# LJacksonPan/RaTrack

Measured on AMD Instinct MI355X. Metric: radar frame-pairs/sec (backbone forward, eval) at B=64,N=256 per GPU, higher is better.
Workload: dtype f32 (2xfp16 split MFMA: three fp16 products per fp32 product, fp32 accumulate, power-of-two scales per matrix and position); 1 GPU; Track4D.backbone forward, B=64 frame-pairs x N=256 points per GPU, S=512 centroids, eval-mode BN, random-init weights, hipGraph=True, batches in flight=4; global_batch=64, parallelism=replicas x1 (no collective on the forward path)

## Files before the change

include/rtk_fused.h:

```cpp
#ifndef RTK_FUSED_H
#define RTK_FUSED_H

#include "rtk_pointnet2.h"

#ifdef __cplusplus
extern "C" {
#endif

#define RTK_MAX_SRC 4
#define RTK_MAX_LAYERS 4

typedef struct {
    const float *ptr;
    int pitch;
    int channels;
    int per_sample;
} rtk_src_t;

#define RTK_LAYER_SPLIT 0x100
typedef struct {
    const float *w_packed;
    const float *bias;
    int cin16, cout16;
    int act;
// ... 82 lines not shown
    float *out;
    int cout, s0, count, out_pitch;
    const float *wt2;
    int s2;
} rtk_gterm_job_t;
RTK_EXPORT int rtk_global_terms(int samples, int cin, const float *g, int njobs, const rtk_gterm_job_t *jobs, float *bcast, int bcast_pitch,
                                int n, rtk_stream_t stream);

#define RTK_COPY_MAX_JOBS 8
typedef struct {
    const void *src;
    void *dst;
    long bytes;
} rtk_copy_job_t;
RTK_EXPORT int rtk_copy_multi(int njobs, const rtk_copy_job_t *jobs, rtk_stream_t stream);

RTK_EXPORT int rtk_to_channel_major(int samples, int n, int channels, const float *src, int src_pitch, int per_sample,
                                    float *dst, int dst_channels, int dst_channel_offset, rtk_stream_t stream);

RTK_EXPORT int rtk_ball_query_pair(int b, int n, int npoint, float radius1, int nsample1, float radius2, int nsample2,
                                   const float *new_xyz, const float *xyz, int *idx1, int *idx2, const int *nuniq,
                                   rtk_stream_t stream);

RTK_EXPORT int rtk_three_nn_masked(int b, int n, int m, const float *unknown, const float *known, float *dist2, int *idx,
                                   const int *unknown_nuniq, const int *known_nuniq, rtk_stream_t stream);

RTK_EXPORT int rtk_geometry_front(int b, int clouds, int n, int npoint, const float *frame1, const float *frame2, int channel_major,
                                  const float *feature1, const float *feature2, float *xyz, float *raw, int *fps_idx, float *new_xyz,
                                  int *nuniq, int *tie, int *first_tie, float *snap, const int *n_valid, int64_t *knn12, int64_t *knn11,
                                  const float *q1_w, float *q1_out, int q1_cout, rtk_stream_t stream);
RTK_EXPORT int rtk_geometry_tables(int samples, int n, int npoint, const float *xyz0, const float *new_xyz, const int *nuniq,
                                   const float *radii, const int *nsamples, int *const *ball, int *const *nn_idx, float *const *nn_dist2,
                                   rtk_stream_t stream);

typedef struct {
    const float *src; float *dst;
    int channels, src_pitch, per_sample, dst_channels, dst_channel_offset;
} rtk_layout_job_t;
RTK_EXPORT int rtk_to_channel_major_multi(int samples, int n, int njobs, const rtk_layout_job_t *jobs, rtk_stream_t stream);

RTK_EXPORT int rtk_log_sinkhorn(int m, int n, const float *scores, float alpha, int iters, float *out, rtk_stream_t stream);

RTK_EXPORT int rtk_dbscan(int n, const float *feat, int pitch, const int *channels, const float *score, float threshold, double eps,
                          int min_samples, int *labels, rtk_stream_t stream);

#define RTK_DESC 141

typedef struct {
    const float *ptr;
    long long sb, sc, sp;
} rtk_bcn_view_t;

typedef struct {
    int B, N;
    rtk_bcn_view_t pc1, flow, feature1, prop, cls;
    const int *n_valid;
    const unsigned char *active;
} rtk_track_frame_t;

#define RTK_DBSCAN_POINT_BYTES 48
RTK_EXPORT int rtk_dbscan_batched(const rtk_track_frame_t *frame, float threshold, double eps, int min_samples, int K, int *labels,
                                  int *obj, int *num_objects, int *flags, void *work, long long work_bytes, rtk_stream_t stream);

RTK_EXPORT int rtk_object_descriptors(const rtk_track_frame_t *frame, int K, const int *obj, const int *num_objects,
                                      const int *prev_count, const float *desc_prev, float *desc, rtk_stream_t stream);

// ... 17 lines not shown
```

ratrack_amd/csrc/ops_pointnet2.hip:

```cpp
#include <math.h>
#include <stdarg.h>
#include <string.h>

#include "rtk_common.h"
#include "rtk_fused.h"

static thread_local char g_err[512] = "";

void rtk_set_error(const char *fmt, ...) {
    va_list ap;
    va_start(ap, fmt);
    vsnprintf(g_err, sizeof(g_err), fmt, ap);
    va_end(ap);
}

extern "C" const char *rtk_last_error(void) { return g_err; }
extern "C" int rtk_version(void) { return (0 << 16) | 3; }

template <int CTRL, int ROW_MASK>
__device__ __forceinline__ unsigned dpp_max_u32(unsigned v) {
    const unsigned o = (unsigned)__builtin_amdgcn_update_dpp(0, (int)v, CTRL, ROW_MASK, 0xf, true);
    return v > o ? v : o;
}

// ... 404 lines not shown
                const float py = USE_LDS ? sy[k] : xyz[k * 3 + 1];
                const float pz = USE_LDS ? sz[k] : xyz[k * 3 + 2];
                hit = rtk_sqdist(qx, qy, qz, px, py, pz) < radius2;
            }
            const unsigned long long mask = __ballot(hit);
            if (mask) {
                if (first < 0) first = base + __builtin_ctzll(mask);
                const int rank = cnt + __builtin_popcountll(mask & ((1ull << lane) - 1ull));
                if (hit && rank < nsample) out[rank] = k;
                cnt += __builtin_popcountll(mask);
            }
        }
        if (first >= 0 && cnt < nsample) {
            for (int l = cnt + lane; l < nsample; l += 64) out[l] = first;
        }
    }
}

extern "C" int rtk_ball_query(int b, int n, int npoint, float radius, int nsample, const float *new_xyz,
                              const float *xyz, int *idx, rtk_stream_t stream) {
    RTK_REQUIRE(b > 0 && n > 0 && npoint > 0 && nsample > 0 && new_xyz && xyz && idx, "ball_query: bad arguments");
    RTK_REQUIRE(b <= 65535, "ball_query: b exceeds grid limits");
    const float r2 = radius * radius;
    dim3 grid(rtk_divup(npoint, BQ_WAVES * BQ_CENTROIDS_PER_WAVE), b);
    const size_t lds = (size_t)n * 3 * sizeof(float);
    if (lds <= 64 * 1024)
        ball_query_kernel<true><<<grid, 64 * BQ_WAVES, lds, (hipStream_t)stream>>>(n, npoint, r2, nsample, new_xyz, xyz, idx);
    else
        ball_query_kernel<false><<<grid, 64 * BQ_WAVES, 0, (hipStream_t)stream>>>(n, npoint, r2, nsample, new_xyz, xyz, idx);
    RTK_CHECK_LAUNCH("ball_query");
    return RTK_OK;
}

__device__ __forceinline__ void ball_query_pair_body(int bs, int chunk0, int chunk_stride, int n, int m, float r2a, int nsa, float r2b, int nsb,
                                                     const float *__restrict__ new_xyz, const float *__restrict__ xyz,
                                                     int *__restrict__ idxa, int *__restrict__ idxb, const int *__restrict__ nuniq,
                                                     float *smem, const int *__restrict__ src_nuniq = nullptr) {
    const int tid = threadIdx.x, wave = tid >> 6, lane = tid & 63;
    constexpr int CPC = BQ_WAVES * BQ_CENTROIDS_PER_WAVE;
    xyz += (size_t)bs * n * 3;
    float *sx = smem, *sy = smem + n, *sz = smem + 2 * n;
    const int climit = nuniq ? min(m, nuniq[bs]) : m;
    if (chunk0 * CPC >= climit) return;
    const int n_full = n;
    if (src_nuniq) n = max(1, min(n, src_nuniq[bs]));
    if (chunk0 == 0) {
        const int z1 = min(m, (climit + 31) & ~31);
        int *za = idxa + ((size_t)bs * m + climit) * nsa, *zb = idxb + ((size_t)bs * m + climit) * nsb;
        for (int l = tid; l < (z1 - climit) * nsa; l += 64 * BQ_WAVES) za[l] = 0;
        for (int l = tid; l < (z1 - climit) * nsb; l += 64 * BQ_WAVES) zb[l] = 0;
    }
    for (int k = tid; k < n; k += 64 * BQ_WAVES) {
        sx[k] = xyz[k * 3 + 0];
        sy[k] = xyz[k * 3 + 1];
        sz[k] = xyz[k * 3 + 2];
    }
    auto fetch = [&](int chunk) {
        const int c0 = (chunk * BQ_WAVES + wave) * BQ_CENTROIDS_PER_WAVE;
        float v = 0.f;
        if (lane < 3 * BQ_CENTROIDS_PER_WAVE && c0 + lane / 3 < climit) v = new_xyz[((size_t)bs * m + c0 + lane / 3) * 3 + lane % 3];
        return v;
    };
    float cq = fetch(chunk0);
    __syncthreads();
    for (int chunk = chunk0; chunk * CPC < climit; chunk += chunk_stride) {
        const int c0 = (chunk * BQ_WAVES + wave) * BQ_CENTROIDS_PER_WAVE;
        const float cq_next = (chunk_stride > 0 && (long)(chunk + chunk_stride) * CPC < climit) ? fetch(chunk + chunk_stride) : 0.f;
        for (int ci = 0; ci < BQ_CENTROIDS_PER_WAVE; ++ci) {
            const int pt = c0 + ci;
            if (pt >= climit) break;
            const float qx = __shfl(cq, 3 * ci, 64), qy = __shfl(cq, 3 * ci + 1, 64), qz = __shfl(cq, 3 * ci + 2, 64);
            int *oa = idxa + ((size_t)bs * m + pt) * nsa;
            int *ob = idxb + ((size_t)bs * m + pt) * nsb;
            int ca = 0, cb = 0, fa = -1, fb = -1;
            bool a0 = false, b0 = false;
            for (int base = 0; base < n && (ca < nsa || cb < nsb); base += 64) {
                const int k = base + lane;
                float d2 = INFINITY;
                if (k < n) d2 = rtk_sqdist(qx, qy, qz, sx[k], sy[k], sz[k]);
                const bool hb = d2 < r2b, ha = d2 < r2a;
                const unsigned long long mb = __ballot(hb);
                if (mb) {
                    const unsigned long long below = (1ull << lane) - 1ull;
                    if (base == 0) b0 = (mb & 1ull) != 0ull;
                    if (cb < nsb) {
                        if (fb < 0) fb = base + __builtin_ctzll(mb);
                        const int rank = cb + __builtin_popcountll(mb & below);
                        if (hb && rank < nsb) ob[rank] = k;
                        cb += __builtin_popcountll(mb);
                    }
                    const unsigned long long ma = __ballot(ha);
                    if (base == 0) a0 = (ma & 1ull) != 0ull;
                    if (ma && ca < nsa) {
                        if (fa < 0) fa = base + __builtin_ctzll(ma);
                        const int rank = ca + __builtin_popcountll(ma & below);
                        if (ha && rank < nsa) oa[rank] = k;
                        ca += __builtin_popcountll(ma);
                    }
                }
            }
            if (n < n_full) {
                if (a0 && ca < nsa) {
                    const int cnt = min(nsa - ca, n_full - n);
                    for (int l = lane; l < cnt; l += 64) oa[ca + l] = n + l;
                    ca += cnt;
                }
                if (b0 && cb < nsb) {
                    const int cnt = min(nsb - cb, n_full - n);
                    for (int l = lane; l < cnt; l += 64) ob[cb + l] = n + l;
                    cb += cnt;
                }
            }
            if (fa >= 0 && ca < nsa) for (int l = ca + lane; l < nsa; l += 64) oa[l] = fa;
            if (fb >= 0 && cb < nsb) for (int l = cb + lane; l < nsb; l += 64) ob[l] = fb;
            if (fa < 0) for (int l = lane; l < nsa; l += 64) oa[l] = 0;
            if (fb < 0) for (int l = lane; l < nsb; l += 64) ob[l] = 0;
        }
        if (chunk_stride <= 0) break;
        cq = cq_next;
    }
}

__global__ __launch_bounds__(64 * BQ_WAVES) void ball_query_pair_kernel(int n, int m, float r2a, int nsa, float r2b, int nsb,
                                                                         const float *__restrict__ new_xyz,
                                                                         const float *__restrict__ xyz, int *__restrict__ idxa,
                                                                         int *__restrict__ idxb, const int *__restrict__ nuniq) {
    extern __shared__ __attribute__((aligned(16))) float smem[];
    ball_query_pair_body(blockIdx.y, blockIdx.x, 0, n, m, r2a, nsa, r2b, nsb, new_xyz, xyz, idxa, idxb, nuniq, smem);
}

extern "C" int rtk_ball_query_pair(int b, int n, int npoint, float radius1, int nsample1, float radius2, int nsample2,
                                   const float *new_xyz, const float *xyz, int *idx1, int *idx2, const int *nuniq,
                                   rtk_stream_t stream) {
    RTK_REQUIRE(b > 0 && n > 0 && npoint > 0 && nsample1 > 0 && nsample2 > 0 && new_xyz && xyz && idx1 && idx2, "ball_query_pair: bad arguments");
    RTK_REQUIRE(radius1 <= radius2, "ball_query_pair: radius1 (%g) must not exceed radius2 (%g)", radius1, radius2);
    RTK_REQUIRE(b <= 65535 && (size_t)n * 12 <= 64 * 1024, "ball_query_pair: b or n too large (n=%d)", n);
    dim3 grid(rtk_divup(npoint, BQ_WAVES * BQ_CENTROIDS_PER_WAVE), b);
    ball_query_pair_kernel<<<grid, 64 * BQ_WAVES, (size_t)n * 12, (hipStream_t)stream>>>(n, npoint, radius1 * radius1, nsample1,
                                                                                         radius2 * radius2, nsample2, new_xyz, xyz,
                                                                                         idx1, idx2, nuniq);
    RTK_CHECK_LAUNCH("ball_query_pair");
    return RTK_OK;
}

__global__ void group_points_kernel(int c, int n, int sn, const float *__restrict__ points,
                                    const int *__restrict__ idx, float *__restrict__ out) {
    const int bs = blockIdx.z, ci = blockIdx.y, t = blockIdx.x * blockDim.x + threadIdx.x;
    if (t >= sn) return;
    out[((size_t)bs * c + ci) * sn + t] = points[((size_t)bs * c + ci) * n + idx[(size_t)bs * sn + t]];
}

__global__ void group_points_grad_kernel(int c, int n, int sn, const float *__restrict__ grad_out,
                                         const int *__restrict__ idx, float *__restrict__ grad_points) {
// ... 160 lines not shown

template <int K, int LPQ = 16>
__device__ __forceinline__ void kv_row_merge(unsigned (&d)[K], int (&i)[K]) {
    unsigned od[K];
    int oi[K];
#pragma unroll
    for (int a = 0; a < K; ++a) { od[a] = dpp_pull<0x101>(d[a]); oi[a] = (int)dpp_pull<0x101>((unsigned)i[a]); }
    kv_merge_low<K>(d, i, od, oi);
#pragma unroll
    for (int a = 0; a < K; ++a) { od[a] = dpp_pull<0x102>(d[a]); oi[a] = (int)dpp_pull<0x102>((unsigned)i[a]); }
    kv_merge_low<K>(d, i, od, oi);
    static_assert(LPQ == 4 || LPQ == 8 || LPQ == 16, "4, 8 or 16 lanes per query");
    if constexpr (LPQ >= 8) {
#pragma unroll
        for (int a = 0; a < K; ++a) { od[a] = dpp_pull<0x104>(d[a]); oi[a] = (int)dpp_pull<0x104>((unsigned)i[a]); }
        kv_merge_low<K>(d, i, od, oi);
    }
    if constexpr (LPQ == 16) {
#pragma unroll
        for (int a = 0; a < K; ++a) { od[a] = dpp_pull<0x108>(d[a]); oi[a] = (int)dpp_pull<0x108>((unsigned)i[a]); }
        kv_merge_low<K>(d, i, od, oi);
    }
}

#ifndef KV_LPQ
#define KV_LPQ 4
#endif
constexpr int KV_QPW = 256 / KV_LPQ;

template <bool USE_LDS>
__device__ __forceinline__ void three_nn_body(int bs, int chunk0, int chunk_stride, int n, int m, const float *__restrict__ unknown,
                                              const float *__restrict__ known, float *__restrict__ dist2,
                                              int *__restrict__ idx, const int *__restrict__ unknown_nuniq,
                                              const int *__restrict__ known_nuniq, float *smem) {
    const int tid = threadIdx.x;
    const int qlimit = unknown_nuniq ? min(n, unknown_nuniq[bs]) : n;
    if (chunk0 * KV_QPW >= qlimit) return;
    const int m_full = m;
    const int ke = known_nuniq ? min(m, known_nuniq[bs]) : m;
    known += (size_t)bs * m * 3;
    m = ke;
    float *sx = smem, *sy = smem + m, *sz = smem + 2 * m;
    const int li = tid & (KV_LPQ - 1);
    auto query = [&](int chunk, float &x, float &y, float &z) {
        const int pr = chunk * KV_QPW + tid / KV_LPQ;
        const float *u = unknown + ((size_t)bs * n + (pr < n ? pr : n - 1)) * 3;
        x = u[0]; y = u[1]; z = u[2];
    };
    float ux, uy, uz;
    query(chunk0, ux, uy, uz);
    if (USE_LDS) {
        for (int k = tid; k < m; k += 256) {
            sx[k] = known[k * 3 + 0];
            sy[k] = known[k * 3 + 1];
            sz[k] = known[k * 3 + 2];
        }
        __syncthreads();
    }
    for (int chunk = chunk0; chunk * KV_QPW < qlimit; chunk += chunk_stride) {
        const int pt_raw = chunk * KV_QPW + tid / KV_LPQ;
        const int pt = pt_raw < n ? pt_raw : n - 1;
        float nx = 0.f, ny = 0.f, nz = 0.f;
        if (chunk_stride > 0 && (chunk + chunk_stride) * KV_QPW < qlimit) query(chunk + chunk_stride, nx, ny, nz);
        unsigned d[4] = {KEY_INF_D, KEY_INF_D, KEY_INF_D, KEY_INF_D};
        int i[4] = {KEY_INF_I, KEY_INF_I, KEY_INF_I, KEY_INF_I};
        for (int k = li; k < m; k += KV_LPQ) {
            const float kx = USE_LDS ? sx[k] : known[k * 3 + 0];
            const float ky = USE_LDS ? sy[k] : known[k * 3 + 1];
            const float kz = USE_LDS ? sz[k] : known[k * 3 + 2];
            const float dd = rtk_sqdist(ux, uy, uz, kx, ky, kz);
            if (dd < INFINITY) {
                d[3] = __float_as_uint(dd); i[3] = k;
                kv_cex(d[2], i[2], d[3], i[3]);
                kv_cex(d[1], i[1], d[2], i[2]);
                kv_cex(d[0], i[0], d[1], i[1]);
            }
        }
        if (li >= 1 && li <= 2 && ke + li - 1 < m_full) {
            const float kx = USE_LDS ? sx[0] : known[0], ky = USE_LDS ? sy[0] : known[1], kz = USE_LDS ? sz[0] : known[2];
            const float dd = rtk_sqdist(ux, uy, uz, kx, ky, kz);
            if (dd < INFINITY) {
                d[3] = __float_as_uint(dd); i[3] = ke + li - 1;
                kv_cex(d[2], i[2], d[3], i[3]);
                kv_cex(d[1], i[1], d[2], i[2]);
                kv_cex(d[0], i[0], d[1], i[1]);
            }
        }
        d[3] = KEY_INF_D; i[3] = KEY_INF_I;
        kv_row_merge<4, KV_LPQ>(d, i);
        if (li == 0 && pt_raw < n) {
            float *od = dist2 + ((size_t)bs * n + pt) * 3;
            int *oi = idx + ((size_t)bs * n + pt) * 3;
#pragma unroll
            for (int a = 0; a < 3; ++a) {
                od[a] = __uint_as_float(d[a]);
                oi[a] = d[a] == KEY_INF_D ? 0 : i[a];
            }
        }
        if (chunk_stride <= 0) break;
        ux = nx; uy = ny; uz = nz;
    }
}

template <bool USE_LDS>
__global__ __launch_bounds__(256) void three_nn_kernel(int n, int m, const float *__restrict__ unknown,
                                                       const float *__restrict__ known, float *__restrict__ dist2,
                                                       int *__restrict__ idx, const int *__restrict__ unknown_nuniq,
                                                       const int *__restrict__ known_nuniq) {
    extern __shared__ __attribute__((aligned(16))) float smem[];
    three_nn_body<USE_LDS>(blockIdx.y, blockIdx.x, 0, n, m, unknown, known, dist2, idx, unknown_nuniq, known_nuniq, smem);
}

extern "C" int rtk_three_nn(int b, int n, int m, const float *unknown, const float *known, float *dist2, int *idx,
                            rtk_stream_t stream) {
    RTK_REQUIRE(b > 0 && n > 0 && m > 0 && unknown && known && dist2 && idx, "three_nn: bad arguments");
    RTK_REQUIRE(b <= 65535, "three_nn: b exceeds grid limits");
    dim3 grid(rtk_divup(n, KV_QPW), b);
    const size_t lds = (size_t)m * 3 * sizeof(float);
    if (lds <= 64 * 1024)
        three_nn_kernel<true><<<grid, 256, lds, (hipStream_t)stream>>>(n, m, unknown, known, dist2, idx, nullptr, nullptr);
    else
        three_nn_kernel<false><<<grid, 256, 0, (hipStream_t)stream>>>(n, m, unknown, known, dist2, idx, nullptr, nullptr);
    RTK_CHECK_LAUNCH("three_nn");
    return RTK_OK;
}

extern "C" int rtk_three_nn_masked(int b, int n, int m, const float *unknown, const float *known, float *dist2, int *idx,
                                   const int *unknown_nuniq, const int *known_nuniq, rtk_stream_t stream) {
    RTK_REQUIRE(b > 0 && n > 0 && m > 0 && unknown && known && dist2 && idx, "three_nn_masked: bad arguments");
// ... 389 lines not shown
                                  const float *feature1, const float *feature2, float *xyz, float *raw, int *fps_idx, float *new_xyz,
                                  int *nuniq, int *tie, int *first_tie, float *snap, const int *n_valid, int64_t *knn12, int64_t *knn11,
                                  const float *q1_w, float *q1_out, int q1_cout, rtk_stream_t stream) {
    RTK_REQUIRE(b > 0 && n > 0 && npoint > 0 && frame1 && fps_idx && new_xyz && nuniq && tie && first_tie && snap,
                "geometry_front: bad arguments (b=%d n=%d npoint=%d)", b, n, npoint);
    RTK_REQUIRE(clouds == b || (clouds == 2 * b && frame2), "geometry_front: clouds=%d must be b or 2 b (b=%d) with both frames", clouds, b);
    RTK_REQUIRE(n <= 2048 && npoint <= 512, "geometry_front: n=%d > 2048 or npoint=%d > 512 (use the separate entry points)", n, npoint);
    RTK_REQUIRE((xyz == nullptr) == (raw == nullptr) && (!xyz || (feature1 && feature2)), "geometry_front: xyz, raw and the features go together");
    RTK_REQUIRE((knn12 == nullptr) == (knn11 == nullptr) && (!knn12 || (n >= 16 && clouds == 2 * b)),
                "geometry_front: the two kNN tables go together (n >= 16, both frames)");
    RTK_REQUIRE((q1_w == nullptr) == (q1_out == nullptr) && (!q1_w || (xyz && q1_cout > 0 && q1_cout % 4 == 0)),
                "geometry_front: q1_w, q1_out go together (with the layout conversion; q1_cout a multiple of 4)");
    GeoFrontParams P;
    P.q1_w = q1_w; P.q1_out = q1_out; P.q1_cout = q1_cout;
    P.B = b; P.S = clouds; P.n = n; P.npoint = npoint; P.block_n = fps_block_size(n); P.block_np = fps_block_size(npoint);
    P.fr1 = frame1; P.fr2 = frame2; P.ps = channel_major ? 1 : 3; P.cs = channel_major ? n : 1;
    P.f1 = feature1; P.f2 = feature2; P.xyz_out = xyz; P.raw_out = raw;
    P.fps_idx = fps_idx; P.new_xyz = new_xyz; P.nuniq = nuniq; P.tie = tie; P.first_tie = first_tie; P.snap = snap; P.n_valid = n_valid;
    P.knn12 = knn12; P.knn11 = knn11; P.knn_chunks = rtk_divup(n, KV_QPW);
    const int grid = clouds + (knn12 ? 2 * b * P.knn_chunks : 0);
    const size_t lds = (size_t)(n > npoint ? n : npoint) * sizeof(float4);
    hipStream_t s = (hipStream_t)stream;
    if (n <= 64 * 4) geometry_front_kernel<4, 8><<<grid, 256, lds, s>>>(P);
    else if (n <= 64 * 8) geometry_front_kernel<8, 8><<<grid, 256, lds, s>>>(P);
    else if (n <= 64 * 16) geometry_front_kernel<16, 8><<<grid, 256, lds, s>>>(P);
    else geometry_front_kernel<32, 8><<<grid, 256, lds, s>>>(P);
    RTK_CHECK_LAUNCH("geometry_front");
    return RTK_OK;
}

#ifndef GEO_TABLES_WGS
#define GEO_TABLES_WGS 2048
#endif
struct GeoBallTask {
    int n_src, nsa, nsb;
    float r2a, r2b;
    const float *new_xyz, *xyz;
    int *idxa, *idxb;
    const int *nuniq, *src_nuniq;
};
struct GeoNnTask {
    int n, m, wgs;
    const float *unknown, *known;
    float *dist2;
    int *idx;
    const int *unknown_nuniq, *known_nuniq;
};
struct GeoTablesParams {
    int samples, npoint, ball_wgs;
    GeoBallTask ball[3];
    GeoNnTask nn[3];
};

__global__ __launch_bounds__(256) void geometry_tables_kernel(const GeoTablesParams P) {
    extern __shared__ __attribute__((aligned(16))) float s_tab[];
    int r = blockIdx.x;
    const int per_ball = P.samples * P.ball_wgs;
    if (r < 3 * per_ball) {
        const int t = r / per_ball, rem = r - t * per_ball, bs = rem / P.ball_wgs, w = rem - bs * P.ball_wgs;
        const GeoBallTask &T = P.ball[t];
        ball_query_pair_body(bs, w, P.ball_wgs, T.n_src, P.npoint, T.r2a, T.nsa, T.r2b, T.nsb, T.new_xyz, T.xyz, T.idxa, T.idxb, T.nuniq, s_tab, T.src_nuniq);
        return;
    }
    r -= 3 * per_ball;
#pragma unroll
    for (int t = 0; t < 3; ++t) {
        const GeoNnTask &T = P.nn[t];
        const int per = P.samples * T.wgs;
        if (r < per) {
            const int bs = r / T.wgs, w = r - bs * T.wgs;
            three_nn_body<true>(bs, w, T.wgs, T.n, T.m, T.unknown, T.known, T.dist2, T.idx, T.unknown_nuniq, T.known_nuniq, s_tab);
            return;
        }
        r -= per;
    }
}

extern "C" int rtk_geometry_tables(int samples, int n, int npoint, const float *xyz0, const float *new_xyz, const int *nuniq,
                                   const float *radii, const int *nsamples, int *const *ball, int *const *nn_idx, float *const *nn_dist2,
                                   rtk_stream_t stream) {
    RTK_REQUIRE(samples > 0 && n > 0 && npoint > 0 && xyz0 && new_xyz && nuniq && radii && nsamples && ball && nn_idx && nn_dist2,
                "geometry_tables: bad arguments");
    const int big = n > npoint ? n : npoint;
    RTK_REQUIRE((size_t)big * 12 <= 64 * 1024, "geometry_tables: clouds of %d points do not fit the LDS stage", big);
    GeoTablesParams P;
    const int want = rtk_divup(GEO_TABLES_WGS, 9 * samples);
    const int ball_chunks = rtk_divup(npoint, BQ_WAVES * BQ_CENTROIDS_PER_WAVE);
    P.samples = samples; P.npoint = npoint; P.ball_wgs = want < ball_chunks ? want : ball_chunks;
    const size_t lv = (size_t)samples * npoint * 3;
    const float *lvl_xyz[4] = {xyz0, new_xyz, new_xyz + lv, new_xyz + 2 * lv};
    const int lvl_n[4] = {n, npoint, npoint, npoint};
    for (int l = 0; l < 3; ++l) {
        RTK_REQUIRE(radii[2 * l] <= radii[2 * l + 1] && nsamples[2 * l] > 0 && nsamples[2 * l + 1] > 0 && ball[2 * l] && ball[2 * l + 1],
                    "geometry_tables: level %d: radii must ascend, tables must be given", l);
        GeoBallTask &T = P.ball[l];
        T.n_src = lvl_n[l]; T.nsa = nsamples[2 * l]; T.nsb = nsamples[2 * l + 1];
        T.r2a = radii[2 * l] * radii[2 * l]; T.r2b = radii[2 * l + 1] * radii[2 * l + 1];
        T.new_xyz = lvl_xyz[l + 1]; T.xyz = lvl_xyz[l]; T.idxa = ball[2 * l]; T.idxb = ball[2 * l + 1]; T.nuniq = nuniq + (size_t)l * samples;
        T.src_nuniq = l > 0 ? nuniq + (size_t)(l - 1) * samples : nullptr;
    }
    const int uk[3][2] = {{2, 3}, {1, 2}, {0, 1}};
    int total = 3 * samples * P.ball_wgs;
    for (int i = 0; i < 3; ++i) {
        const int u = uk[i][0], k = uk[i][1];
        RTK_REQUIRE(nn_idx[i] && nn_dist2[i], "geometry_tables: three-NN table %d missing", i);
        GeoNnTask &T = P.nn[i];
        T.n = lvl_n[u]; T.m = lvl_n[k]; T.wgs = want < rtk_divup(T.n, KV_QPW) ? want : rtk_divup(T.n, KV_QPW);
        T.unknown = lvl_xyz[u]; T.known = lvl_xyz[k]; T.dist2 = nn_dist2[i]; T.idx = nn_idx[i];
        T.unknown_nuniq = u > 0 ? nuniq + (size_t)(u - 1) * samples : nullptr;
        T.known_nuniq = nuniq + (size_t)(k - 1) * samples;
        total += samples * T.wgs;
    }
    geometry_tables_kernel<<<total, 256, (size_t)big * 12, (hipStream_t)stream>>>(P);
    RTK_CHECK_LAUNCH("geometry_tables");
    return RTK_OK;
}
```

ratrack_amd/fused.py:

```python
import ctypes
import os

import torch

from . import _lib
from . import pointnet2_hip as _native

ACT_NONE, ACT_RELU, ACT_LEAKY, ACT_SIGMOID = 0, 1, 2, 3


class _Src(ctypes.Structure):
    _fields_ = [("ptr", ctypes.c_void_p), ("pitch", ctypes.c_int), ("channels", ctypes.c_int), ("per_sample", ctypes.c_int)]


class _Layer(ctypes.Structure):
    _fields_ = [("w_packed", ctypes.c_void_p), ("bias", ctypes.c_void_p), ("cin16", ctypes.c_int), ("cout16", ctypes.c_int),
                ("act", ctypes.c_int), ("inv_scale", ctypes.c_float)]


class _Interp(ctypes.Structure):
    _fields_ = [("known_feats", ctypes.c_void_p), ("pitch", ctypes.c_int), ("channels", ctypes.c_int), ("m", ctypes.c_int),
                ("idx", ctypes.c_void_p), ("dist2", ctypes.c_void_p), ("nuniq", ctypes.c_void_p)]


_vp, _ci = ctypes.c_void_p, ctypes.c_int
_lib.SIGNATURES.update({
    "rtk_pointwise_mlp": [_ci, _ci, ctypes.POINTER(_Interp), _ci, ctypes.POINTER(_Src), _vp, _ci, ctypes.POINTER(_Layer), _vp,
                          _ci, _ci, _ci, _vp, _vp, _vp],
    "rtk_pointwise_mlp_tap": [_ci, _ci, ctypes.POINTER(_Interp), ctypes.POINTER(_Layer), _vp, _ci, _vp, ctypes.POINTER(_Layer), _ci, _vp, _ci,
                              _vp],
    "rtk_sa_scale": [_ci] * 4 + [_vp] * 4 + [_ci, _ci, _vp, _ci, ctypes.POINTER(_Layer), _vp, _ci, _ci, _vp, _vp, _vp],
    "rtk_cost_volume": [_ci] * 3 + [_vp] * 6 + [ctypes.POINTER(_Layer), ctypes.POINTER(_Layer), _vp, _ci, _vp],
    "rtk_patch_cost": [_ci] * 2 + [_vp] * 3 + [_ci, ctypes.POINTER(_Layer), _vp, _ci, _ci, _vp],
    "rtk_pack_split_layer": [_ci, _ci, _vp, _ci, _vp, _vp, _vp],
    "rtk_cost_volume_split": [_ci] * 3 + [_vp] * 10 + [ctypes.POINTER(_Layer), _vp, _ci, _vp],
    "rtk_cost_volume_split_shared": [_ci] * 3 + [_vp] * 10 + [ctypes.POINTER(_Layer), _vp, _ci, _ci, _vp],
    "rtk_cost_volume_split_term": [_ci] * 3 + [_vp] * 11 + [ctypes.POINTER(_Layer), _vp, _ci, _ci, _vp],
    "rtk_split_mlp2": [_ci, _vp, _vp, _vp, _vp, _vp, _vp, _vp],
    "rtk_sa_scale_split": [_ci] * 4 + [_vp] * 4 + [_ci, _ci, _vp, _vp, _vp, _vp, _vp, _ci, _ci, _vp, _vp, _vp],
    "rtk_prepare_inputs": [_ci] * 2 + [_vp] * 6 + [_vp],
    "rtk_fps_centroids": [_ci] * 3 + [_vp] * 8 + [_vp],
    "rtk_knn_point_masked": [_ci] * 4 + [_vp] * 4 + [_vp],
    "rtk_fps_relevel": [_ci] * 3 + [_vp] * 9 + [_ci, _vp, _vp],
    "rtk_gru_step": [_ci] * 3 + [_vp] * 8 + [_vp],
    "rtk_to_channel_major": [_ci] * 3 + [_vp, _ci, _ci, _vp, _ci, _ci, _vp],
    "rtk_ball_query_pair": [_ci] * 3 + [ctypes.c_float, _ci, ctypes.c_float, _ci] + [_vp] * 5 + [_vp],
    "rtk_geometry_front": [_ci] * 4 + [_vp, _vp, _ci] + [_vp] * 13 + [_vp, _vp, _ci, _vp],
    "rtk_geometry_tables": [_ci] * 3 + [_vp] * 3 + [ctypes.POINTER(ctypes.c_float), ctypes.POINTER(_ci), ctypes.POINTER(_vp), ctypes.POINTER(_vp),
                            ctypes.POINTER(_vp), _vp],
    "rtk_three_nn_masked": [_ci] * 3 + [_vp] * 6 + [_vp],
    "rtk_to_channel_major_multi": [_ci] * 3 + [_vp, _vp],
    "rtk_log_sinkhorn": [_ci, _ci, _vp, ctypes.c_float, _ci, _vp, _vp],
    "rtk_dbscan": [_ci, _vp, _ci, _vp, _vp, ctypes.c_float, ctypes.c_double, _ci, _vp, _vp],
    "rtk_dbscan_batched": [_vp, ctypes.c_float, ctypes.c_double, _ci, _ci, _vp, _vp, _vp, _vp, _vp, ctypes.c_longlong, _vp],
    "rtk_object_descriptors": [_vp, _ci, _vp, _vp, _vp, _vp, _vp, _vp],
    "rtk_affinity_pairs": [_ci, _ci] + [_vp] * 7 + [_vp],
    "rtk_associate_batched": [_ci] * 3 + [_vp] * 7 + [ctypes.c_float, _ci] + [_vp] * 9 + [_vp],
    "rtk_track_max_objects": [],
})


class _GtJob(ctypes.Structure):
    _fields_ = [("wt", ctypes.c_void_p), ("bias", ctypes.c_void_p), ("out", ctypes.c_void_p), ("cout", ctypes.c_int), ("s0", ctypes.c_int),
                ("count", ctypes.c_int), ("out_pitch", ctypes.c_int), ("wt2", ctypes.c_void_p), ("s2", ctypes.c_int)]


class _CopyJob(ctypes.Structure):
    _fields_ = [("src", ctypes.c_void_p), ("dst", ctypes.c_void_p), ("bytes", ctypes.c_long)]


_lib.SIGNATURES.update({
    "rtk_gru_step_head": [_ci] * 3 + [_vp] * 11 + [_ci, _vp],
    "rtk_global_terms": [_ci, _ci, _vp, _ci, ctypes.POINTER(_GtJob), _vp, _ci, _ci, _vp],
    "rtk_copy_multi": [_ci, ctypes.POINTER(_CopyJob), _vp],
})


def copy_multi(pairs):
    for i in range(0, len(pairs), 8):
        part = pairs[i:i + 8]
        jobs = (_CopyJob * len(part))()
        for j, (d, s_) in enumerate(part):
# ... 270 lines not shown
            w2 = ws[1][0].float().to(device).contiguous()
            self.split_bias = ws[1][1].float().to(device).contiguous()
            self.split_image, self.split_scale = pack_split_device(w2)
            torch.cuda.current_stream().synchronize()


class _PNHeadWeights:

    RADII = [[2, 4], [4, 8], [8, 16]]
    NSAMPLES = [[4, 8], [8, 16], [16, 32]]

    def __init__(self, sd, prefix, device):
        d = lambda k: sd[prefix + k].double()
        self.scales = [[_SAScale(sd, "%ssa%d.mlps.%d" % (prefix, l + 1, s), self.NSAMPLES[l][s], self.RADII[l][s], device)
                        for s in range(2)] for l in range(3)]
        self.wq1 = torch.cat([self.scales[0][0].wf, self.scales[0][1].wf], 0)
        self.trans = []
        for l in (1, 2):
            wl, bl = d("linear%d.weight" % l), d("linear%d.bias" % l)
            rows, bias = [wl], [bl]
            for s in range(2):
                wf = self.scales[l][s].wf
                rows.append(wf @ wl)
                bias.append(wf @ bl)
            self.trans.append(Chain([(torch.cat(rows, 0), torch.cat(bias, 0), ACT_NONE)], device))
        self.lin3 = Chain([(d("linear3.weight"), d("linear3.bias"), ACT_NONE)], device)
        self.fp = {}
        for name in ("fp3", "fp2", "fp1"):
            w, b = fold_bn(sd[prefix + name + ".mlp.layer0.conv.weight"], prefix + name + ".mlp.layer0.bn.bn", sd)
            self.fp[name] = Chain([(w, b, ACT_RELU)], device)


FUSED_GEOMETRY = True
GEOMETRY_POISON = None
CHECK_FPS_RELEVEL = False


def check_fps_relevel(xyz1, idx, new_xyz, nuniq):
    S_, npoint, _ = xyz1.shape
    src = xyz1
    for l in range(idx.shape[0]):
        i = torch.empty(S_, npoint, dtype=torch.int32, device=src.device)
        out = torch.empty(S_, npoint, 3, dtype=torch.float32, device=src.device)
        cnt = torch.empty(S_, dtype=torch.int32, device=src.device)
        _lib.call("rtk_fps_centroids", S_, npoint, npoint, src.data_ptr(), i.data_ptr(), out.data_ptr(), cnt.data_ptr(), None, None, None, None,
                  _stream())
        assert torch.equal(i, idx[l].view(S_, npoint)), "fps_relevel: level %d indices differ from the full selection" % (l + 2)
        assert torch.equal(out, new_xyz[l].view(S_, npoint, 3)), "fps_relevel: level %d centroids differ" % (l + 2)
        assert torch.equal(cnt, nuniq[l].view(-1)), "fps_relevel: level %d exhausted-cloud counters differ" % (l + 2)
        src = out


class _NullCtx:
    def __enter__(self):
        return self

    def __exit__(self, *a):
        return False


class Geometry:

    def __init__(self, xyz, npoint, side=None, knn_frames=0, finite=False, n_valid=None, level_hook=None, tail_hook=None, zeros=None,
                 prepare=None, q1=None):
        zeros_given = zeros
        zeros = zeros or (lambda n_, dtype, device: torch.zeros(n_, dtype=dtype, device=device))
# ... 43 lines not shown
        main = torch.cuda.current_stream()
        if side is not None:
            side.wait_stream(main)
        ctx = torch.cuda.stream(side) if side is not None else _NullCtx()
        self.ball = [[ball[lvl * 2 + s].view(S_, npoint, _PNHeadWeights.NSAMPLES[lvl][s]) for s in range(2)] for lvl in range(3)]
        if fused_geo:
            with ctx:
                for lvl in range(3):
                    self.xyz.append(new_xyz[lvl])
                    self.nuniq.append(cnt[lvl])
                b1 = S_ // 2 if (B or prepare is not None) else S_
                if prepare is not None:
                    pc1, pc2, f1, f2, raw = prepare
                    fr = (pc1.data_ptr(), pc2.data_ptr(), 1, f1.data_ptr(), f2.data_ptr(), xyz.data_ptr(), raw.data_ptr())
                    self._scratch = self._scratch + (pc1, pc2, f1, f2, raw)
                else:
                    fr = (xyz.data_ptr(), xyz[b1:].data_ptr() if b1 < S_ else None, 0, None, None, None, None)
                _lib.call("rtk_geometry_front", b1, S_, n, npoint, *fr, fps_idx[0].data_ptr(), xyz_all.data_ptr(), cnt[0].data_ptr(),
                          tie.data_ptr(), first_tie.data_ptr(), snap.data_ptr(), nv, self.knn[0].data_ptr() if B else None,
                          self.knn[1].data_ptr() if B else None, q1[0].data_ptr() if q1w else None, q1[1].data_ptr() if q1w else None,
                          q1[1].shape[1] if q1w else 0, _stream())
                self.q1_done = q1w
                self._record("front", side)
                if CHECK_FPS_RELEVEL and not torch.cuda.is_current_stream_capturing():
                    check_fps_relevel(new_xyz[0], torch.stack(self.fps_idx[1:]), xyz_all[1:], torch.stack(list(cnt[1:3])))
                radii = (ctypes.c_float * 6)(*[float(r) for row in _PNHeadWeights.RADII for r in row])
                nsam = (_ci * 6)(*ns_all)
                balls = (_vp * 6)(*[t.data_ptr() for t in ball])
                self.nn = {}
                for i, (name, (u, k)) in enumerate({"fp3": (2, 3), "fp2": (1, 2), "fp1": (0, 1)}.items()):
                    self.nn[name] = (d2_parts[i].view(S_, nn_rows[i], 3), nn_idx[i].view(S_, nn_rows[i], 3), self.xyz[k].shape[1])
                nni = (_vp * 3)(*[self.nn[k][1].data_ptr() for k in ("fp3", "fp2", "fp1")])
                nnd = (_vp * 3)(*[self.nn[k][0].data_ptr() for k in ("fp3", "fp2", "fp1")])
                _lib.call("rtk_geometry_tables", S_, n, npoint, xyz.data_ptr(), xyz_all.data_ptr(), cnt[0].data_ptr(), radii, nsam, balls, nni, nnd,
                          _stream())
                for lvl in range(3):
                    if level_hook is not None:
                        level_hook(self, lvl)
                    self._record(lvl, side)
                self._record("nn", side)
                if B:
                    self.events["knn"] = self.events.get("front")
                if tail_hook is not None:
                    tail_hook(self)
            return
        with ctx:
            if not big:
                _lib.call("rtk_fps_centroids", S_, n, npoint, xyz.data_ptr(), fps_idx[0].data_ptr(), new_xyz[0].data_ptr(),
                          cnt[0].data_ptr(), tie.data_ptr(), nv, snap.data_ptr(), first_tie.data_ptr(), _stream())
            else:
                _native.furthest_point_sampling_wrapper(S_, n, npoint, xyz, temp, self.fps_idx[0])
                new_xyz[0].copy_(torch.gather(xyz, 1, self.fps_idx[0].long().unsqueeze(-1).expand(-1, -1, 3)))
                cnt[0].fill_(npoint)
                tie.fill_(npoint)

            def relevel():
                resume = (fps_idx[0].data_ptr(), snap.data_ptr(), n, first_tie.data_ptr()) if not big else (None, None, 0, None)
                _lib.call("rtk_fps_relevel", S_, npoint, 2, new_xyz[0].data_ptr(), cnt[0].data_ptr(), tie.data_ptr(),
                          fps_idx[1].data_ptr(), new_xyz[1].data_ptr(), cnt[1].data_ptr(), tie23[0].data_ptr(), *resume, _stream())
                if CHECK_FPS_RELEVEL and not torch.cuda.is_current_stream_capturing():
                    check_fps_relevel(new_xyz[0], torch.stack(self.fps_idx[1:]), xyz_all[1:], torch.stack(list(cnt[1:3])))
            for lvl in range(3):
                self.xyz.append(new_xyz[lvl])
                self.nuniq.append(cnt[lvl])
            self.ball = []
            for lvl in range(3):
                row = []
                for s in range(2):
# ... 474 lines not shown
```

Before: 105,100 frame-pairs/s.

## Share ball-query and three-NN tables across levels when FPS levels coincide

```diff
diff --git a/include/rtk_fused.h b/include/rtk_fused.h
--- a/include/rtk_fused.h
+++ b/include/rtk_fused.h
@@ -138,6 +138,9 @@
 RTK_EXPORT int rtk_geometry_tables(int samples, int n, int npoint, const float *xyz0, const float *new_xyz, const int *nuniq,
                                    const float *radii, const int *nsamples, int *const *ball, int *const *nn_idx, float *const *nn_dist2,
                                    rtk_stream_t stream);
+RTK_EXPORT int rtk_geometry_tables_shared(int samples, int n, int npoint, const float *xyz0, const float *new_xyz, const int *nuniq,
+                                          const int *tie, const float *radii, const int *nsamples, int *const *ball, int *const *nn_idx,
+                                          float *const *nn_dist2, rtk_stream_t stream);
 
 typedef struct {
     const float *src; float *dst;
diff --git a/ratrack_amd/csrc/ops_pointnet2.hip b/ratrack_amd/csrc/ops_pointnet2.hip
--- a/ratrack_amd/csrc/ops_pointnet2.hip
+++ b/ratrack_amd/csrc/ops_pointnet2.hip
@@ -460,10 +460,17 @@
     return RTK_OK;
 }
 
-__device__ __forceinline__ void ball_query_pair_body(int bs, int chunk0, int chunk_stride, int n, int m, float r2a, int nsa, float r2b, int nsb,
-                                                     const float *__restrict__ new_xyz, const float *__restrict__ xyz,
-                                                     int *__restrict__ idxa, int *__restrict__ idxb, const int *__restrict__ nuniq,
-                                                     float *smem, const int *__restrict__ src_nuniq = nullptr) {
+template <int NR>
+struct BallScan {
+    float r2[NR];
+    int ns[NR];
+    int *idx[NR], *also_idx[NR];
+};
+
+template <int NR>
+__device__ __forceinline__ void ball_query_multi_body(int bs, int chunk0, int chunk_stride, int n, int m, const BallScan<NR> &S,
+                                                      const float *__restrict__ new_xyz, const float *__restrict__ xyz,
+                                                      const int *__restrict__ nuniq, float *smem, const int *__restrict__ src_nuniq = nullptr) {
     const int tid = threadIdx.x, wave = tid >> 6, lane = tid & 63;
     constexpr int CPC = BQ_WAVES * BQ_CENTROIDS_PER_WAVE;
     xyz += (size_t)bs * n * 3;
@@ -474,9 +481,14 @@
     if (src_nuniq) n = max(1, min(n, src_nuniq[bs]));
     if (chunk0 == 0) {
         const int z1 = min(m, (climit + 31) & ~31);
-        int *za = idxa + ((size_t)bs * m + climit) * nsa, *zb = idxb + ((size_t)bs * m + climit) * nsb;
-        for (int l = tid; l < (z1 - climit) * nsa; l += 64 * BQ_WAVES) za[l] = 0;
-        for (int l = tid; l < (z1 - climit) * nsb; l += 64 * BQ_WAVES) zb[l] = 0;
+#pragma unroll
+        for (int j = 0; j < NR; ++j) {
+            const size_t z0 = ((size_t)bs * m + climit) * S.ns[j];
+            for (int l = tid; l < (z1 - climit) * S.ns[j]; l += 64 * BQ_WAVES) {
+                S.idx[j][z0 + l] = 0;
+                if (S.also_idx[j]) S.also_idx[j][z0 + l] = 0;
+            }
+        }
     }
     for (int k = tid; k < n; k += 64 * BQ_WAVES) {
         sx[k] = xyz[k * 3 + 0];
@@ -498,55 +510,71 @@
             const int pt = c0 + ci;
             if (pt >= climit) break;
             const float qx = __shfl(cq, 3 * ci, 64), qy = __shfl(cq, 3 * ci + 1, 64), qz = __shfl(cq, 3 * ci + 2, 64);
-            int *oa = idxa + ((size_t)bs * m + pt) * nsa;
-            int *ob = idxb + ((size_t)bs * m + pt) * nsb;
-            int ca = 0, cb = 0, fa = -1, fb = -1;
-            bool a0 = false, b0 = false;
-            for (int base = 0; base < n && (ca < nsa || cb < nsb); base += 64) {
+            int *o[NR], *o2[NR];
+            int c[NR], f[NR];
+            bool z[NR];
+#pragma unroll
+            for (int j = 0; j < NR; ++j) {
+                const size_t row = ((size_t)bs * m + pt) * S.ns[j];
+                o[j] = S.idx[j] + row;
+                o2[j] = S.also_idx[j] ? S.also_idx[j] + row : nullptr;
+                c[j] = 0; f[j] = -1; z[j] = false;
+            }
+            auto put = [&](int j, int l, int v) {
+                o[j][l] = v;
+                if (o2[j]) o2[j][l] = v;
+            };
+            auto open = [&]() {
+                bool any = false;
+#pragma unroll
+                for (int j = 0; j < NR; ++j) any |= c[j] < S.ns[j];
+                return any;
+            };
+            for (int base = 0; base < n && open(); base += 64) {
                 const int k = base + lane;
                 float d2 = INFINITY;
                 if (k < n) d2 = rtk_sqdist(qx, qy, qz, sx[k], sy[k], sz[k]);
-                const bool hb = d2 < r2b, ha = d2 < r2a;
-                const unsigned long long mb = __ballot(hb);
-                if (mb) {
+                unsigned long long mk = __ballot(d2 < S.r2[NR - 1]);
+                if (mk) {
                     const unsigned long long below = (1ull << lane) - 1ull;
-                    if (base == 0) b0 = (mb & 1ull) != 0ull;
-                    if (cb < nsb) {
-                        if (fb < 0) fb = base + __builtin_ctzll(mb);
-                        const int rank = cb + __builtin_popcountll(mb & below);
-                        if (hb && rank < nsb) ob[rank] = k;
-                        cb += __builtin_popcountll(mb);
-                    }
-                    const unsigned long long ma = __ballot(ha);
-                    if (base == 0) a0 = (ma & 1ull) != 0ull;
-                    if (ma && ca < nsa) {
-                        if (fa < 0) fa = base + __builtin_ctzll(ma);
-                        const int rank = ca + __builtin_popcountll(ma & below);
-                        if (ha && rank < nsa) oa[rank] = k;
-                        ca += __builtin_popcountll(ma);
+#pragma unroll
+                    for (int j = NR - 1; j >= 0; --j) {
+                        const bool h = d2 < S.r2[j];
+                        if (j < NR - 1) mk = __ballot(h);
+                        if (!mk) break;
+                        if (base == 0) z[j] = (mk & 1ull) != 0ull;
+                        if (c[j] < S.ns[j]) {
+                            if (f[j] < 0) f[j] = base + __builtin_ctzll(mk);
+                            const int rank = c[j] + __builtin_popcountll(mk & below);
+                            if (h && rank < S.ns[j]) put(j, rank, k);
+                            c[j] += __builtin_popcountll(mk);
+                        }
                     }
                 }
             }
-            if (n < n_full) {
-                if (a0 && ca < nsa) {
-                    const int cnt = min(nsa - ca, n_full - n);
-                    for (int l = lane; l < cnt; l += 64) oa[ca + l] = n + l;
-                    ca += cnt;
+#pragma unroll
+            for (int j = 0; j < NR; ++j) {
+                const int ns = S.ns[j];
+                if (n < n_full && z[j] && c[j] < ns) {
+                    const int cnt = min(ns - c[j], n_full - n);
+                    for (int l = lane; l < cnt; l += 64) put(j, c[j] + l, n + l);
+                    c[j] += cnt;
                 }
-                if (b0 && cb < nsb) {
-                    const int cnt = min(nsb - cb, n_full - n);
-                    for (int l = lane; l < cnt; l += 64) ob[cb + l] = n + l;
-                    cb += cnt;
-                }
-            }
-            if (fa >= 0 && ca < nsa) for (int l = ca + lane; l < nsa; l += 64) oa[l] = fa;
-            if (fb >= 0 && cb < nsb) for (int l = cb + lane; l < nsb; l += 64) ob[l] = fb;
-            if (fa < 0) for (int l = lane; l < nsa; l += 64) oa[l] = 0;
-            if (fb < 0) for (int l = lane; l < nsb; l += 64) ob[l] = 0;
+                if (f[j] >= 0 && c[j] < ns) for (int l = c[j] + lane; l < ns; l += 64) put(j, l, f[j]);
+                if (f[j] < 0) for (int l = lane; l < ns; l += 64) put(j, l, 0);
+            }
         }
         if (chunk_stride <= 0) break;
         cq = cq_next;
     }
+}
+
+__device__ __forceinline__ void ball_query_pair_body(int bs, int chunk0, int chunk_stride, int n, int m, float r2a, int nsa, float r2b, int nsb,
+                                                     const float *__restrict__ new_xyz, const float *__restrict__ xyz,
+                                                     int *__restrict__ idxa, int *__restrict__ idxb, const int *__restrict__ nuniq,
+                                                     float *smem, const int *__restrict__ src_nuniq = nullptr) {
+    const BallScan<2> S = {{r2a, r2b}, {nsa, nsb}, {idxa, idxb}, {nullptr, nullptr}};
+    ball_query_multi_body<2>(bs, chunk0, chunk_stride, n, m, S, new_xyz, xyz, nuniq, smem, src_nuniq);
 }
 
 __global__ __launch_bounds__(64 * BQ_WAVES) void ball_query_pair_kernel(int n, int m, float r2a, int nsa, float r2b, int nsb,
@@ -773,7 +801,8 @@
 __device__ __forceinline__ void three_nn_body(int bs, int chunk0, int chunk_stride, int n, int m, const float *__restrict__ unknown,
                                               const float *__restrict__ known, float *__restrict__ dist2,
                                               int *__restrict__ idx, const int *__restrict__ unknown_nuniq,
-                                              const int *__restrict__ known_nuniq, float *smem) {
+                                              const int *__restrict__ known_nuniq, float *smem, float *__restrict__ also_dist2 = nullptr,
+                                              int *__restrict__ also_idx = nullptr) {
     const int tid = threadIdx.x;
     const int qlimit = unknown_nuniq ? min(n, unknown_nuniq[bs]) : n;
     if (chunk0 * KV_QPW >= qlimit) return;
@@ -836,6 +865,15 @@
             for (int a = 0; a < 3; ++a) {
                 od[a] = __uint_as_float(d[a]);
                 oi[a] = d[a] == KEY_INF_D ? 0 : i[a];
+            }
+            if (also_idx) {
+                float *od2 = also_dist2 + ((size_t)bs * n + pt) * 3;
+                int *oi2 = also_idx + ((size_t)bs * n + pt) * 3;
+#pragma unroll
+                for (int a = 0; a < 3; ++a) {
+                    od2[a] = __uint_as_float(d[a]);
+                    oi2[a] = d[a] == KEY_INF_D ? 0 : i[a];
+                }
             }
         }
         if (chunk_stride <= 0) break;
@@ -1291,8 +1329,11 @@
 #ifndef GEO_TABLES_WGS
 #define GEO_TABLES_WGS 2048
 #endif
+#ifndef GEO_TABLES_STANDBY_WGS
+#define GEO_TABLES_STANDBY_WGS 1
+#endif
 struct GeoBallTask {
-    int n_src, nsa, nsb;
+    int n_src, nsa, nsb, wgs;
     float r2a, r2b;
     const float *new_xyz, *xyz;
     int *idxa, *idxb;
@@ -1306,71 +1347,138 @@
     const int *unknown_nuniq, *known_nuniq;
 };
 struct GeoTablesParams {
-    int samples, npoint, ball_wgs;
+    int samples, npoint;
     GeoBallTask ball[3];
     GeoNnTask nn[3];
+    const int *tie;
 };
+
+template <bool SHARED>
+__device__ __forceinline__ void geometry_tables_body(const GeoTablesParams &P, float *s_tab) {
+    int r = blockIdx.x, bs = 0, w = 0;
+    auto mine = [&](int wgs) {
+        const int per = P.samples * wgs;
+        if (r < per) { bs = r / wgs; w = r - bs * wgs; return true; }
+        r -= per;
+        return false;
+    };
+    auto ball = [&](const GeoBallTask &T) {
+        ball_query_pair_body(bs, w, T.wgs, T.n_src, P.npoint, T.r2a, T.nsa, T.r2b, T.nsb, T.new_xyz, T.xyz, T.idxa, T.idxb, T.nuniq, s_tab, T.src_nuniq);
+    };
+    auto nn = [&](const GeoNnTask &T, float *also_dist2, int *also_idx) {
+        three_nn_body<true>(bs, w, T.wgs, T.n, T.m, T.unknown, T.known, T.dist2, T.idx, T.unknown_nuniq, T.known_nuniq, s_tab, also_dist2, also_idx);
+    };
+    if (SHARED) {
+        int bt = -1, nt = -1;
+        if (mine(P.ball[2].wgs)) {
+            if (P.tie[bs] == 0) return;
+            bt = 2;
+        } else if (mine(P.nn[0].wgs)) {
+            if (P.tie[bs] == 0) return;
+            nt = 0;
+        } else if (mine(P.ball[1].wgs)) {
+            if (P.tie[bs] == 0) {
+                const GeoBallTask &T = P.ball[1], &U = P.ball[2];
+                const BallScan<3> S = {{T.r2a, T.r2b, U.r2b}, {T.nsa, T.nsb, U.nsb}, {T.idxa, T.idxb, U.idxb}, {nullptr, U.idxa, nullptr}};
+                ball_query_multi_body<3>(bs, w, T.wgs, T.n_src, P.npoint, S, T.new_xyz, T.xyz, T.nuniq, s_tab, T.src_nuniq);
+                return;
+            }
+            bt = 1;
+        } else if (mine(P.ball[0].wgs)) {
+            bt = 0;
+        } else if (mine(P.nn[1].wgs)) {
+            nt = 1;
+        } else if (mine(P.nn[2].wgs)) {
+            nt = 2;
+        } else {
+            return;
+        }
+        if (bt >= 0) {
+            ball(P.ball[bt]);
+        } else {
+            const bool both = nt == 1 && P.tie[bs] == 0;
+            nn(P.nn[nt], both ? P.nn[0].dist2 : nullptr, both ? P.nn[0].idx : nullptr);
+        }
+        return;
+    }
+    const int per_ball = P.samples * P.ball[0].wgs;
+    if (r < 3 * per_ball) {
+        const int t = r / per_ball;
+        r -= t * per_ball;
+        mine(P.ball[0].wgs);
+        ball(P.ball[t]);
+        return;
+    }
+    r -= 3 * per_ball;
+#pragma unroll
+    for (int t = 0; t < 3; ++t)
+        if (mine(P.nn[t].wgs)) { nn(P.nn[t], nullptr, nullptr); return; }
+}
 
 __global__ __launch_bounds__(256) void geometry_tables_kernel(const GeoTablesParams P) {
     extern __shared__ __attribute__((aligned(16))) float s_tab[];
-    int r = blockIdx.x;
-    const int per_ball = P.samples * P.ball_wgs;
-    if (r < 3 * per_ball) {
-        const int t = r / per_ball, rem = r - t * per_ball, bs = rem / P.ball_wgs, w = rem - bs * P.ball_wgs;
-        const GeoBallTask &T = P.ball[t];
-        ball_query_pair_body(bs, w, P.ball_wgs, T.n_src, P.npoint, T.r2a, T.nsa, T.r2b, T.nsb, T.new_xyz, T.xyz, T.idxa, T.idxb, T.nuniq, s_tab, T.src_nuniq);
-        return;
-    }
-    r -= 3 * per_ball;
-#pragma unroll
-    for (int t = 0; t < 3; ++t) {
-        const GeoNnTask &T = P.nn[t];
-        const int per = P.samples * T.wgs;
-        if (r < per) {
-            const int bs = r / T.wgs, w = r - bs * T.wgs;
-            three_nn_body<true>(bs, w, T.wgs, T.n, T.m, T.unknown, T.known, T.dist2, T.idx, T.unknown_nuniq, T.known_nuniq, s_tab);
-            return;
-        }
-        r -= per;
-    }
-}
-
-extern "C" int rtk_geometry_tables(int samples, int n, int npoint, const float *xyz0, const float *new_xyz, const int *nuniq,
-                                   const float *radii, const int *nsamples, int *const *ball, int *const *nn_idx, float *const *nn_dist2,
-                                   rtk_stream_t stream) {
+    geometry_tables_body<false>(P, s_tab);
+}
+
+__global__ __launch_bounds__(256) void geometry_tables_shared_kernel(const GeoTablesParams P) {
+    extern __shared__ __attribute__((aligned(16))) float s_tab[];
+    geometry_tables_body<true>(P, s_tab);
+}
+
+static int geometry_tables_launch(int samples, int n, int npoint, const float *xyz0, const float *new_xyz, const int *nuniq,
+                                  const float *radii, const int *nsamples, int *const *ball, int *const *nn_idx, float *const *nn_dist2,
+                                  const int *tie, rtk_stream_t stream) {
     RTK_REQUIRE(samples > 0 && n > 0 && npoint > 0 && xyz0 && new_xyz && nuniq && radii && nsamples && ball && nn_idx && nn_dist2,
                 "geometry_tables: bad arguments");
     const int big = n > npoint ? n : npoint;
     RTK_REQUIRE((size_t)big * 12 <= 64 * 1024, "geometry_tables: clouds of %d points do not fit the LDS stage", big);
     GeoTablesParams P;
-    const int want = rtk_divup(GEO_TABLES_WGS, 9 * samples);
+    const bool shared = tie && radii[3] == radii[4] && nsamples[3] == nsamples[4] && radii[2] <= radii[3] && radii[3] <= radii[5];
+    const int want = rtk_divup(GEO_TABLES_WGS, (shared ? 7 : 9) * samples);
     const int ball_chunks = rtk_divup(npoint, BQ_WAVES * BQ_CENTROIDS_PER_WAVE);
-    P.samples = samples; P.npoint = npoint; P.ball_wgs = want < ball_chunks ? want : ball_chunks;
+    P.samples = samples; P.npoint = npoint; P.tie = shared ? tie : nullptr;
     const size_t lv = (size_t)samples * npoint * 3;
     const float *lvl_xyz[4] = {xyz0, new_xyz, new_xyz + lv, new_xyz + 2 * lv};
     const int lvl_n[4] = {n, npoint, npoint, npoint};
+    int total = 0;
     for (int l = 0; l < 3; ++l) {
         RTK_REQUIRE(radii[2 * l] <= radii[2 * l + 1] && nsamples[2 * l] > 0 && nsamples[2 * l + 1] > 0 && ball[2 * l] && ball[2 * l + 1],
                     "geometry_tables: level %d: radii must ascend, tables must be given", l);
         GeoBallTask &T = P.ball[l];
-        T.n_src = lvl_n[l]; T.nsa = nsamples[2 * l]; T.nsb = nsamples[2 * l + 1];
+        const int w = (shared && l == 2) ? GEO_TABLES_STANDBY_WGS : want;
+        T.n_src = lvl_n[l]; T.nsa = nsamples[2 * l]; T.nsb = nsamples[2 * l + 1]; T.wgs = w < ball_chunks ? w : ball_chunks;
         T.r2a = radii[2 * l] * radii[2 * l]; T.r2b = radii[2 * l + 1] * radii[2 * l + 1];
         T.new_xyz = lvl_xyz[l + 1]; T.xyz = lvl_xyz[l]; T.idxa = ball[2 * l]; T.idxb = ball[2 * l + 1]; T.nuniq = nuniq + (size_t)l * samples;
         T.src_nuniq = l > 0 ? nuniq + (size_t)(l - 1) * samples : nullptr;
+        total += samples * T.wgs;
     }
     const int uk[3][2] = {{2, 3}, {1, 2}, {0, 1}};
-    int total = 3 * samples * P.ball_wgs;
     for (int i = 0; i < 3; ++i) {
         const int u = uk[i][0], k = uk[i][1];
         RTK_REQUIRE(nn_idx[i] && nn_dist2[i], "geometry_tables: three-NN table %d missing", i);
         GeoNnTask &T = P.nn[i];
-        T.n = lvl_n[u]; T.m = lvl_n[k]; T.wgs = want < rtk_divup(T.n, KV_QPW) ? want : rtk_divup(T.n, KV_QPW);
+        const int w = (shared && i == 0) ? GEO_TABLES_STANDBY_WGS : want;
+        T.n = lvl_n[u]; T.m = lvl_n[k]; T.wgs = w < rtk_divup(T.n, KV_QPW) ? w : rtk_divup(T.n, KV_QPW);
         T.unknown = lvl_xyz[u]; T.known = lvl_xyz[k]; T.dist2 = nn_dist2[i]; T.idx = nn_idx[i];
         T.unknown_nuniq = u > 0 ? nuniq + (size_t)(u - 1) * samples : nullptr;
         T.known_nuniq = nuniq + (size_t)(k - 1) * samples;
         total += samples * T.wgs;
     }
-    geometry_tables_kernel<<<total, 256, (size_t)big * 12, (hipStream_t)stream>>>(P);
+    if (shared) geometry_tables_shared_kernel<<<total, 256, (size_t)big * 12, (hipStream_t)stream>>>(P);
+    else geometry_tables_kernel<<<total, 256, (size_t)big * 12, (hipStream_t)stream>>>(P);
     RTK_CHECK_LAUNCH("geometry_tables");
     return RTK_OK;
 }
+
+extern "C" int rtk_geometry_tables(int samples, int n, int npoint, const float *xyz0, const float *new_xyz, const int *nuniq,
+                                   const float *radii, const int *nsamples, int *const *ball, int *const *nn_idx, float *const *nn_dist2,
+                                   rtk_stream_t stream) {
+    return geometry_tables_launch(samples, n, npoint, xyz0, new_xyz, nuniq, radii, nsamples, ball, nn_idx, nn_dist2, nullptr, stream);
+}
+
+extern "C" int rtk_geometry_tables_shared(int samples, int n, int npoint, const float *xyz0, const float *new_xyz, const int *nuniq,
+                                          const int *tie, const float *radii, const int *nsamples, int *const *ball, int *const *nn_idx,
+                                          float *const *nn_dist2, rtk_stream_t stream) {
+    RTK_REQUIRE(tie, "geometry_tables_shared: the tie words of rtk_geometry_front are missing");
+    return geometry_tables_launch(samples, n, npoint, xyz0, new_xyz, nuniq, radii, nsamples, ball, nn_idx, nn_dist2, tie, stream);
+}
diff --git a/ratrack_amd/fused.py b/ratrack_amd/fused.py
--- a/ratrack_amd/fused.py
+++ b/ratrack_amd/fused.py
@@ -48,6 +48,8 @@
     "rtk_geometry_front": [_ci] * 4 + [_vp, _vp, _ci] + [_vp] * 13 + [_vp, _vp, _ci, _vp],
     "rtk_geometry_tables": [_ci] * 3 + [_vp] * 3 + [ctypes.POINTER(ctypes.c_float), ctypes.POINTER(_ci), ctypes.POINTER(_vp), ctypes.POINTER(_vp),
                             ctypes.POINTER(_vp), _vp],
+    "rtk_geometry_tables_shared": [_ci] * 3 + [_vp] * 4 + [ctypes.POINTER(ctypes.c_float), ctypes.POINTER(_ci), ctypes.POINTER(_vp),
+                                   ctypes.POINTER(_vp), ctypes.POINTER(_vp), _vp],
     "rtk_three_nn_masked": [_ci] * 3 + [_vp] * 6 + [_vp],
     "rtk_to_channel_major_multi": [_ci] * 3 + [_vp, _vp],
     "rtk_log_sinkhorn": [_ci, _ci, _vp, ctypes.c_float, _ci, _vp, _vp],
@@ -384,6 +386,7 @@
 
 
 FUSED_GEOMETRY = True
+SHARED_TABLES = True
 GEOMETRY_POISON = None
 CHECK_FPS_RELEVEL = False
 
@@ -493,8 +496,12 @@
                     self.nn[name] = (d2_parts[i].view(S_, nn_rows[i], 3), nn_idx[i].view(S_, nn_rows[i], 3), self.xyz[k].shape[1])
                 nni = (_vp * 3)(*[self.nn[k][1].data_ptr() for k in ("fp3", "fp2", "fp1")])
                 nnd = (_vp * 3)(*[self.nn[k][0].data_ptr() for k in ("fp3", "fp2", "fp1")])
-                _lib.call("rtk_geometry_tables", S_, n, npoint, xyz.data_ptr(), xyz_all.data_ptr(), cnt[0].data_ptr(), radii, nsam, balls, nni, nnd,
-                          _stream())
+                if SHARED_TABLES:
+                    _lib.call("rtk_geometry_tables_shared", S_, n, npoint, xyz.data_ptr(), xyz_all.data_ptr(), cnt[0].data_ptr(), tie.data_ptr(),
+                              radii, nsam, balls, nni, nnd, _stream())
+                else:
+                    _lib.call("rtk_geometry_tables", S_, n, npoint, xyz.data_ptr(), xyz_all.data_ptr(), cnt[0].data_ptr(), radii, nsam, balls, nni,
+                              nnd, _stream())
                 for lvl in range(3):
                     if level_hook is not None:
                         level_hook(self, lvl)
```

Result: no change. 105,800 frame-pairs/s (median of 6 runs) (+0.7%).
